# DreamWaterFound/self_commit_ORB-SLAM2

Hardware: AMD Instinct MI355X
Metric: frames/s ORB extract+match (1000 feat, 640x480) (higher is better)
Workload: dtype u8; 1 GPU; batch of 256 synthetic 640x480 frames per GPU (8 distinct resident batches per step, one launch set per batch), ORB extract (1000 feat, 8 levels, FAST 20/7) + brute-force Hamming SearchByBoW of consecutive frames; batch_per_gpu=256, streams=3, width=640, height=480, nfeatures=1000, parallelism=frames sharded, 1 rank(s), no data-path collective

## Files before the change

### self_commit_orb-slam2_amd/csrc/orbx_extractor.hip

```cpp
#include <math.h>
#include <stdarg.h>
#include <stdio.h>
#include <stdlib.h>
#include <string.h>

#include <algorithm>
#include <atomic>
#include <chrono>
#include <condition_variable>
#include <functional>
#include <memory>
#include <mutex>
#include <thread>
#include <vector>

#include "orbx_internal.h"

static thread_local char g_err[512] = "";

void orbx_set_error(const char *fmt, ...)
{
    va_list ap;
    va_start(ap, fmt);
    vsnprintf(g_err, sizeof(g_err), fmt, ap);
// ... 49 lines not shown
    hipStream_t stream = nullptr;
    hipEvent_t ev[ORBX_PROF_RING][ST_COUNT + 1] = {};
    bool profiling = false;
    int profCount = 0;
    bool debugTaps = false;
    DevBuf<OrbxGeom> geomDev;
    DevBuf<uint8_t> binDev, pyr, blur, score, staging;
    DevBuf<uint32_t> rsDev;
    DevBuf<OrbxFcCell> fcDev;
    DevBuf<int> cellCount, lvlCnt, lvlBase, status;
    DevBuf<uint8_t> outArena[2];
    int *outCntP[2] = {nullptr, nullptr};
    int *outStP[2] = {nullptr, nullptr};
    orbx_keypoint *outKpP[2] = {nullptr, nullptr};
    uint8_t *outDescP[2] = {nullptr, nullptr};
    size_t arenaKpOff = 0, arenaDescOff = 0, arenaBytes = 0;
    hipEvent_t consumerEv[2] = {nullptr, nullptr};
    hipEvent_t pyrConsumerEv = nullptr;
    int cur = 0;
    DevBuf<uint32_t> cellSlots, ptBuf, labBuf;
    DevBuf<OrbxLevelKp> lvlKp;
    int allocBatch = 0;
    int lastBatch = 0;
    bool lastChunked = false;
    const uint8_t *lastImg0 = nullptr;
    int lastStride = 0;
    size_t lastFramePitch = 0;
    uint8_t *hostStaging = nullptr;
    size_t hostStagingBytes = 0;
    int stagingStride = 0;
    size_t stagingFramePitch = 0;
    uint8_t *hostOut = nullptr;
    size_t hostOutBytes = 0;
    hipGraph_t sgGraph[2] = {nullptr, nullptr};
    hipGraphExec_t sgExec[2] = {nullptr, nullptr};
    bool sgValid = false;
    bool sgDisabled = false;
    struct Combiner *comb = nullptr;
    bool combDisabled = false;
    orbx_extractor *expectPartner = nullptr;
    bool isEngine = false;
    size_t hostPyrOff = 0;
    bool hostPyrValid = false;
    bool hostSynced = false;
    bool lastCombined = false;
    struct PipeSlot {
// ... 214 lines not shown
    g.fcPitch = maxWCell <= 32 ? 48 : maxWCell <= 48 ? 64 : 80;
    g.fcScPitch = maxWCell <= 42 ? 48 : 80;
    {
        int maxAw = 1;
        for (int l = 0; l < nl; l++) {
            const OrbxLevel &lv = g.lv[l];
            const int maxBX = lv.w - ORBX_BORDER;
            for (int cj = 0; cj < lv.nCols; cj++) {
                const int iniX = ORBX_BORDER + cj * lv.wCell, maxX = std::min(iniX + lv.wCell + 6, maxBX);
                maxAw = std::max(maxAw, (maxX - 3) - (iniX + 3));
            }
        }
        g.fcScPitch = maxAw + 2 <= 48 ? 48 : 80;
        if (g.fcScPitch == 80) g.fcPitch = 80;
    }
    { const char *pe = getenv("ORBX_FC_PITCH"); if (pe && atoi(pe) == 80 && g.fcPitch == 64) g.fcPitch = 80; }
    {
        const int units = (maxHCell + 6) * ((maxWCell + 6 + 15) / 16), ns = (units + 63) / 64;
        g.fcNS = ns <= 2 ? 2 : ns <= 3 ? 3 : ns <= 4 ? 4 : 6;
    }
    g.fcInBytes = g.fcPitch * (maxHCell + 6);
    g.fcScBytes = g.fcScPitch * (maxHCell + 2);
    g.fcLdsBytes = g.fcInBytes + g.fcScBytes + (int)align_up((size_t)maxWCell * maxHCell * 2, 16);
    h->fcHost.assign((size_t)cells, OrbxFcCell{});
    for (int l = 0; l < nl; l++) {
        const OrbxLevel &lv = g.lv[l];
        const int maxBX = lv.w - ORBX_BORDER, maxBY = lv.h - ORBX_BORDER;
        for (int ci = 0; ci < lv.nRows; ci++)
            for (int cj = 0; cj < lv.nCols; cj++) {
                const int cell = ci * lv.nCols + cj;
                OrbxFcCell &e = h->fcHost[(size_t)lv.cellBase + cell];
                const int iniX = ORBX_BORDER + cj * lv.wCell, iniY = ORBX_BORDER + ci * lv.hCell;
                const int maxX = std::min(iniX + lv.wCell + 6, maxBX), maxY = std::min(iniY + lv.hCell + 6, maxBY);
                const int x0 = iniX + 3, x1 = maxX - 3, y0 = iniY + 3, y1 = maxY - 3, aw = x1 - x0, ah = y1 - y0;
                const bool valid = !(iniY >= maxBY - 3 || iniX >= maxBX - 6 || aw <= 0 || ah <= 0);
                e.xy = valid ? ((uint32_t)x0 | ((uint32_t)y0 << 16)) : ((uint32_t)ORBX_EDGE | ((uint32_t)ORBX_EDGE << 16));
                const int ew = valid ? aw : 1, eh = valid ? ah : 1, nu = (ew + 6 + 15) / 16;
                e.dim = (uint32_t)ew | ((uint32_t)eh << 8) | ((uint32_t)l << 16) | (valid ? 1u << 24 : 0u);
                e.inv = (uint32_t)((65536 + nu - 1) / nu); e.units = (uint32_t)nu | ((uint32_t)((eh + 6) * nu) << 8);
                e.pitch = lv.pitch; e.off = (uint32_t)lv.off;
                e.slot = (uint32_t)(lv.slotBase + cell * lv.cellCap); e.cap = (uint32_t)lv.cellCap;
            }
    }
    g.pyrBytes = align_up(off + 256, 256);
    if (maxNodes > 2048) { orbx_set_error("per-level feature quota %d exceeds the quadtree node capacity 2048", maxNodes); return ORBX_ERR_ARG; }
    h->nodeCap = maxNodes <= 256 ? 256 : (maxNodes <= 512 ? 512 : (maxNodes <= 1024 ? 1024 : 2048));
// ... 100 lines not shown
    if (h->pyrConsumerEv) { ORBX_HIP_CHECK(hipStreamWaitEvent(h->stream, h->pyrConsumerEv, 0)); h->pyrConsumerEv = nullptr; }
    ORBX_HIP_CHECK(hipMemsetAsync(h->status.p, 0, (size_t)(batch + 1) * sizeof(int), h->stream));
    if (prof) ORBX_HIP_CHECK(hipEventRecord(ev[0], h->stream));
    static const bool batchTiles = getenv("ORBX_BATCH_PYR_TILES") && getenv("ORBX_BATCH_PYR_TILES")[0] == '1';
    bool tiled = false;
    if (batchTiles && h->allocBatch > 1) {
        if (h->ptBatchW != W || h->ptBatchH != H) {
            std::vector<OrbxPyrTile> plan;
            h->ptTiles = 0;
            if (plan_pyramid_tiles(h, plan, h->ptTiles, h->ptLds, h->ptTab)) {
                if ((rc = h->ptDev.ensure(plan.size())) != ORBX_OK) return rc;
                ORBX_HIP_CHECK(hipMemcpy(h->ptDev.p, plan.data(), plan.size() * sizeof(OrbxPyrTile), hipMemcpyHostToDevice));
            } else h->ptTiles = 0;
            h->ptBatchW = W; h->ptBatchH = H;
        }
        if (h->ptTiles > 0) {
            L.pyrTiles = h->ptDev.p; L.pyrTileCount = h->ptTiles; L.pyrTileBuf = h->ptLds; L.pyrTileTab = h->ptTab;
            if ((rc = orbx_launch_pyramid_tiles(L)) != ORBX_OK) return rc;
            tiled = true;
        }
    }
    const char *es = getenv("ORBX_PYR_SPLIT");
    L.pyrBand = !tiled && h->geom.pyrBand && !(es && es[0] == '1');
    if (L.pyrBand) {
        for (int l = 0; l < h->geom.nlevels; l++)
            if ((rc = orbx_launch_pyr_band(L, l)) != ORBX_OK) return rc;
    } else if (!tiled)
        for (int l = 1; l < h->geom.nlevels; l++)
            if ((rc = orbx_launch_resize(L, l)) != ORBX_OK) return rc;
    if (prof) ORBX_HIP_CHECK(hipEventRecord(ev[ST_PYR + 1], h->stream));
    if ((rc = orbx_launch_fast_cells(L)) != ORBX_OK) return rc;
    if (prof) ORBX_HIP_CHECK(hipEventRecord(ev[ST_FAST + 1], h->stream));
    if ((rc = orbx_launch_octree(L)) != ORBX_OK) return rc;
    if (prof) ORBX_HIP_CHECK(hipEventRecord(ev[ST_OCTREE + 1], h->stream));
    if (prof) ORBX_HIP_CHECK(hipEventRecord(ev[ST_ORIENT + 1], h->stream));
    if (!L.pyrBand && (rc = orbx_launch_blur(L)) != ORBX_OK) return rc;
    if (prof) ORBX_HIP_CHECK(hipEventRecord(ev[ST_BLUR + 1], h->stream));
    if (h->consumerEv[cb]) { ORBX_HIP_CHECK(hipStreamWaitEvent(h->stream, h->consumerEv[cb], 0)); h->consumerEv[cb] = nullptr; }
    if ((rc = orbx_launch_orient_describe(L)) != ORBX_OK) return rc;
    if (prof) { ORBX_HIP_CHECK(hipEventRecord(ev[ST_DESC + 1], h->stream)); h->profCount++; }
    h->lastBatch = batch; h->lastImg0 = img0Dev; h->lastStride = stride; h->lastFramePitch = framePitch;
    h->lastCombined = false; h->hostSynced = false; h->lastChunked = false;
    return ORBX_OK;
}

static int host_copy_threads()
{
    static const int n = [] {
        const char *e = getenv("ORBX_HOST_COPY_THREADS");
        int v = e && *e ? atoi(e) : (int)std::min(16u, std::max(1u, std::thread::hardware_concurrency() / 2));
        return v < 1 ? 1 : v > 64 ? 64 : v;
    }();
    return n;
}
struct CopyPool {
    std::mutex m;
    std::mutex jm;
    std::condition_variable cvWork, cvDone;
    std::vector<std::thread> workers;
    std::function<void(int, int)> job;
    int n = 0, parts = 0, gen = 0, pending = 0;
    bool stop = false;
    void worker(int id)
    {
        int seen = 0;
        for (;;) {
            std::function<void(int, int)> fn;
// ... 1514 lines not shown
```

### self_commit_orb-slam2_amd/csrc/orbx_internal.h

```cpp
#ifndef ORBX_INTERNAL_H
#define ORBX_INTERNAL_H

#include <hip/hip_runtime.h>
#include <cstring>
#include <stdint.h>

#include "../../include/orbx.h"

#define ORBX_MAX_LEVELS 12
#define ORBX_EDGE 19
#define ORBX_BORDER 16
#define ORBX_HALF_PATCH 15
#define ORBX_PATCH 31
#define ORBX_CELL_W 30
#define ORBX_MAX_INI 8

#define ORBX_DEV_ERR_PTCAP 1
#define ORBX_DEV_ERR_NODECAP 2
#define ORBX_DEV_ERR_KPCAP 4

struct OrbxLevel {
    int w, h, pitch;
    int off;
    int nCols, nRows, wCell, hCell;
// ... 4 lines not shown
    int nIni;
    int iniX[ORBX_MAX_INI + 1];
    int binOff;
    int kpBase, kpCap;
    int blurTileBase, blurTilesX, blurTilesY;
    int bandH, bandPitch;
    int bandOff;
    uint32_t bandDivNc, bandDivG4;
    double rsScaleX, rsScaleY;
    int rsColOff, rsRowOff;
    int patchSize;
    float scale;
};

struct OrbxGeom {
    int nlevels, W, H;
    int iniTh, minTh;
    int cellsPerFrame, slotsPerFrame, kpPerFrame, outCap;
    int blurTiles;
    int fcPitch, fcScPitch, fcNS;
    int fcInBytes, fcScBytes, fcLdsBytes;
    size_t pyrBytes;
    int pyrBand;
    uint32_t taps[7];
    int umax[16];
    OrbxLevel lv[ORBX_MAX_LEVELS];
};

#define ORBX_BAND_MAX_ITEMS (1 << 14)
static inline uint32_t orbx_band_div(int n)
{
    uint32_t S = 14;
    while ((1u << (S - 14)) < (uint32_t)n) S++;
    const uint32_t m = (uint32_t)((((uint64_t)1 << S) + (uint64_t)n - 1) / (uint64_t)n);
    return m | (S << 20);
}

struct OrbxFcCell {
    uint32_t xy;
    uint32_t dim;
    int32_t pitch;
    uint32_t off;
    uint32_t slot;
    uint32_t cap;
    uint32_t inv;
    uint32_t units;
};
#define ORBX_FC_CELLS_PER_WAVE 4

struct OrbxPyrTile { short cx0, cy0, cx1, cy1, ox0, oy0, ox1, oy1; };

struct OrbxCombMember {
    const uint8_t *srcImg;
    uint8_t *devImg;
    uint8_t *devPyr;
    uint8_t *devArena;
    uint8_t *hostOut;
    uint8_t *hostPyr;
// ... 4 lines not shown
void orbx_set_error(const char *fmt, ...);
#define ORBX_HIP_CHECK(expr)                                                                           \
    do {                                                                                               \
        hipError_t e_ = (expr);                                                                        \
        if (e_ != hipSuccess) {                                                                        \
            orbx_set_error("%s failed: %s (%s:%d)", #expr, hipGetErrorString(e_), __FILE__, __LINE__); \
            return ORBX_ERR_HIP;                                                                       \
        }                                                                                              \
    } while (0)

struct OrbxLaunch {
    hipStream_t stream;
    const OrbxGeom *geomDev;
    const OrbxGeom *geom;
    int batch;
    const uint8_t *img0;
    int img0Stride;
    size_t img0FramePitch;
    uint8_t *pyr, *blur, *score;
    size_t blurBytes;
    const uint8_t *binTab;
    const uint32_t *rsTab;
    const OrbxFcCell *fcCells;
    int *cellCount;
    uint32_t *cellSlots;
    uint32_t *ptBuf, *labBuf;
    OrbxLevelKp *lvlKp;
    int *lvlCnt;
    int *outBase;
    orbx_keypoint *outKp;
    uint8_t *outDesc;
    int *outCnt;
    int *status;
    int *outStatus;
    int nodeCap;
    bool pyrBand = false;
    const OrbxCombMember *combTab = nullptr;
    OrbxCombMember *combTabCopy = nullptr;
    unsigned *combSync = nullptr;
    unsigned long long *combFlag = nullptr;
    size_t combKpOff = 0, combDescOff = 0;
    const OrbxPyrTile *pyrTiles = nullptr; int pyrTileCount = 0, pyrTileBuf = 0, pyrTileTab = 0;
    hipGraph_t graph = nullptr;
    hipGraphNode_t deps[2] = {nullptr, nullptr};
    int ndeps = 0;
    hipGraphNode_t *node = nullptr;
};

int orbx_launch_resize(const OrbxLaunch &L, int level);
int orbx_launch_pyr_band(const OrbxLaunch &L, int level);
int orbx_launch_pyramid_tiles(const OrbxLaunch &L);
int orbx_launch_comb_upload(const OrbxLaunch &L, uint8_t *stagingDev);
int orbx_launch_comb_finish(const OrbxLaunch &L);
int orbx_launch_fast_cells(const OrbxLaunch &L);
int orbx_launch_octree(const OrbxLaunch &L);
int orbx_launch_blur(const OrbxLaunch &L);
int orbx_launch_octree_blur(const OrbxLaunch &L, bool *fused);
int orbx_launch_gather_frames(hipStream_t stream, const uint8_t *const *framesPinnedTab, int batch, int W, int H, int srcStride, uint8_t *dst, int dstStride, size_t framePitch, bool aligned16);
int orbx_launch_orient_describe(const OrbxLaunch &L);

hipStream_t orbx_extractor_stream_internal(orbx_extractor *h);
bool orbx_extractor_host_complete_internal(orbx_extractor *h, int *status);
int orbx_extractor_host_count_internal(orbx_extractor *h);
const orbx_keypoint *orbx_extractor_host_keypoints_internal(orbx_extractor *h);
void orbx_extractor_set_consumer_event_internal(orbx_extractor *h, hipEvent_t ev);
const int *orbx_extractor_status_word_internal(orbx_extractor *h);


template <typename T> struct OrbxDevBuf {
    T *p = nullptr;
    size_t n = 0;
    int ensure(size_t count)
    {
// ... 158 lines not shown
```

### self_commit_orb-slam2_amd/csrc/orbx_kernels.hip

```cpp
#include <algorithm>
#include "orbx_internal.h"

namespace {

struct OdTables {
    float pat[256][4];
    uint32_t disc[64][4];
};
constexpr int8_t kPattern[1024] = {
#include "orb_pattern.inc"
};
constexpr int kUmax[16] = {15, 15, 15, 15, 14, 14, 14, 13, 13, 12, 11, 10, 9, 8, 6, 3};
constexpr OdTables make_od_tables()
{
    OdTables t{};
    for (int i = 0; i < 256; i++) {
        t.pat[i][0] = (float)kPattern[4 * i]; t.pat[i][2] = (float)kPattern[4 * i + 1];
        t.pat[i][1] = (float)kPattern[4 * i + 2]; t.pat[i][3] = (float)kPattern[4 * i + 3];
    }
    for (int ml = 0; ml < 64; ml++)
        for (int j = 0; j < 4; j++) {
            const int mr = ml >> 1, mh = ml & 1;
            uint32_t m = 0u;
            if (mr < 31) {
// ... 271 lines not shown
                                            0x0c000c00u | (uint32_t)((b) & 3) | ((uint32_t)(((b) & 3) + 1) << 16))


#define FC_STAMP(i) do { if (PROF) { const unsigned long long t_ = __builtin_amdgcn_s_memtime(); pacc[i] += t_ - tPrev; tPrev = __builtin_amdgcn_s_memtime(); pacc[11] += tPrev - t_; } } while (0)

__device__ __forceinline__ uint4 load16u(const uint8_t *p)
{
    typedef uint32_t u32x4_u __attribute__((ext_vector_type(4), aligned(1)));
    const u32x4_u v = *(const u32x4_u *)p;
    return make_uint4(v.x, v.y, v.z, v.w);
}

__device__ __forceinline__ int wave_incl_scan_dpp(int v)
{
    v += __builtin_amdgcn_update_dpp(0, v, 0x111, 0xf, 0xf, false);
    v += __builtin_amdgcn_update_dpp(0, v, 0x112, 0xf, 0xf, false);
    v += __builtin_amdgcn_update_dpp(0, v, 0x114, 0xf, 0xf, false);
    v += __builtin_amdgcn_update_dpp(0, v, 0x118, 0xf, 0xf, false);
    v += __builtin_amdgcn_update_dpp(0, v, 0x142, 0xa, 0xf, false);
    v += __builtin_amdgcn_update_dpp(0, v, 0x143, 0xc, 0xf, false);
    return v;
}

template <int P, int SP, int NS, bool PROF = false, bool DBG = false>
__global__ __launch_bounds__(64) void k_fast_cells(const OrbxFcCell *__restrict__ cells, int K, int cellsPerFrame, int slotsPerFrame, size_t pyrBytes, int iniTh, int minTh,
                                                   int inBytes, int scBytes, const uint8_t *__restrict__ img0, int img0Stride, size_t img0FramePitch,
                                                   const uint8_t *__restrict__ pyr, uint8_t *__restrict__ scoreDbg, int *__restrict__ cellCount,
                                                   uint32_t *__restrict__ cellSlots, unsigned long long *__restrict__ prof)
{
    extern __shared__ __attribute__((aligned(16))) uint8_t lds[];
    uint8_t *inT = lds;
    uint8_t *scT = lds + inBytes;
    unsigned short *cand = (unsigned short *)(scT + scBytes);
    unsigned long long pacc[12] = {0, 0, 0, 0, 0, 0, 0, 0, 0, 0, 0, 0}, tPrev = 0;
    if (PROF) tPrev = __builtin_amdgcn_s_memtime();
    XCD_REMAP_XY(bx, f);
    const int lane = threadIdx.x;
    const int cFirst = bx * K, cEnd = min(cFirst + K, cellsPerFrame);
    const uint8_t *frame0 = img0 + (size_t)f * img0FramePitch, *frameP = pyr + (size_t)f * pyrBytes;
    uint4 wv[NS];
    int wo[NS], ur[NS], uc[NS];
    uint32_t shape = 0xffffffffu;
#define FC_REQUEST(E) do { \
        const int lvl_ = (int)(((E).dim >> 16) & 0xffu), sp_ = lvl_ ? (E).pitch : img0Stride; \
        const uint8_t *base_ = (lvl_ ? frameP + (E).off : frame0) + (size_t)((int)((E).xy >> 16) - 3) * sp_ + ((int)((E).xy & 0xffffu) - 3); \
        if ((E).units != shape) { \
            shape = (E).units; \
            const int nu_ = (int)((E).units & 0xffu), ntot_ = (int)((E).units >> 8), inv_ = (int)(E).inv; \
            _Pragma("unroll") for (int k_ = 0; k_ < NS; k_++) { \
                const int u_ = min(lane + 64 * k_, ntot_ - 1); \
                ur[k_] = __mul24(u_, inv_) >> 16; uc[k_] = 16 * (u_ - __mul24(ur[k_], nu_)); \
                wo[k_] = lane + 64 * k_ < ntot_ ? ur[k_] * P + uc[k_] : -1; \
            } \
        } \
        _Pragma("unroll") for (int k_ = 0; k_ < NS; k_++) wv[k_] = load16u(base_ + (size_t)ur[k_] * sp_ + uc[k_]); \
    } while (0)
    OrbxFcCell e = cells[cFirst], en = cells[min(cFirst + 1, cEnd - 1)];
    FC_REQUEST(e);
    FC_STAMP(0);
    for (int ci = cFirst; ci < cEnd; ci++) {
    int pNc1 = 0, pNc2 = 0, pRetry = 0;
    const int aw = (int)(e.dim & 0xffu), ah = (int)((e.dim >> 8) & 0xffu);
    const bool valid = (e.dim >> 24) != 0;
    const int x0 = (int)(e.xy & 0xffffu), y0 = (int)(e.xy >> 16);
    const int lpitch = e.pitch, cellCap = (int)e.cap;
    const uint32_t loff = e.off, slotOff = e.slot;
    int *cnt = cellCount + (size_t)f * cellsPerFrame + ci;
    {
#pragma unroll
        for (int k = 0; k < NS; k++)
            if (wo[k] >= 0) *(uint4 *)(inT + wo[k]) = wv[k];
        uint4 *z = (uint4 *)scT;
        for (int i = lane; i < (ah + 2) * (SP / 16); i += 64) z[i] = make_uint4(0u, 0u, 0u, 0u);
    }
    e = en;
    FC_REQUEST(e);
    en = cells[min(ci + 2, cEnd - 1)];
    if (!valid) {
        if (lane == 0) *cnt = 0;
        continue;
    }
    __syncthreads();
    FC_STAMP(1);
    uint8_t *dbg = DBG && scoreDbg ? scoreDbg + (size_t)f * pyrBytes + loff : nullptr;
    if (dbg)
        for (int p = lane; p < aw * ah; p += 64) dbg[(size_t)(y0 + p / aw) * lpitch + (x0 + p % aw)] = 0;

    const int S = (aw + 15) >> 4;
    const int rpp = S == 1 ? 64 : S == 2 ? 32 : S == 3 ? 21 : 16;
    const int rl = S == 1 ? lane : S == 2 ? (lane >> 1) : S == 3 ? ((lane * 43) >> 7) : (lane >> 2);
    const int seg = lane - rl * S, c0 = 16 * seg;
    const uint32_t colMask = (aw - c0 >= 16) ? 0xffffu : (aw - c0 <= 0 ? 0u : ((1u << (aw - c0)) - 1u));
    int nc = 0, th = dbg ? minTh : iniTh, base = 0;
    bool anyIni = false;
    uint32_t *slot = cellSlots + (size_t)f * slotsPerFrame + slotOff;
    for (;;) {
    nc = 0;
    const uint32_t thrPk = (uint32_t)(th & 0xffff) * 0x00010001u;
    for (int rowBase = 0; rowBase < ah; rowBase += rpp) {
        const int r = rowBase + rl;
        const bool live = rl < rpp && r < ah;
        const uint8_t *wp = inT + min(r, ah - 1) * P + c0;
        uint32_t W[7][6];
#pragma unroll
        for (int dy = 0; dy < 7; dy += 3) {
// ... 11 lines not shown
                const uint32_t xb = FC_PAIR(W[3 + FAST_DY(k + 8)], j + 3 + FAST_DX(k + 8));
                A = pk_max_u16(A, pk_min_u16(xa, xb));
                B = pk_min_u16(B, pk_max_u16(xa, xb));
            }
            const uint32_t vv = FC_PAIR(W[3], j + 3);
            const uint32_t m = pk_max_i16(pk_sub_i16(vv, A), pk_sub_i16(B, vv));
            mask |= ((pk_sub_i16(thrPk, m) >> 15) & 0x00010001u) << j;
        }
        mask = (mask & 0x5555u) | ((mask >> 15) & 0xaaaau);
        mask = live ? (mask & colMask) : 0u;
        if (PROF) { asm volatile("" :: "v"(mask)); FC_STAMP(th == iniTh || dbg ? 2 : 6); }
        const int cntL = __popc(mask);
        const int incl = wave_incl_scan_dpp(cntL);
        unsigned short *o = cand + (nc + incl - cntL);
        const int code0 = (r << 6) | c0;
        while (mask) {
            const int bpos = __ffs(mask) - 1;
            mask &= mask - 1;
            *o++ = (unsigned short)(code0 + bpos);
        }
        nc += __builtin_amdgcn_readlane(incl, 63);
        FC_STAMP(th == iniTh || dbg ? 3 : 7);
    }
    __syncthreads();
    if (PROF) { if (th == iniTh || dbg) pNc1 = nc; else { pNc2 = nc; pRetry = 1; } }

    for (int i = lane; i < nc; i += 64) {
        const int code = cand[i], r = code >> 6, c = code & 63;
        const uint8_t *q = inT + r * P + c;
        const int v = q[3 * P + 3];
        int x[16];
#pragma unroll
        for (int k = 0; k < 16; k++) x[k] = q[(3 + FAST_DY(k)) * P + 3 + FAST_DX(k)];
        int a3[16], b3[16];
#pragma unroll
        for (int k = 0; k < 16; k++) {
            a3[k] = min3u_asm(x[k], x[(k + 1) & 15], x[(k + 2) & 15]);
            b3[k] = max3u_asm(x[k], x[(k + 1) & 15], x[(k + 2) & 15]);
        }
        int maxA = 0, minB = 255;
#pragma unroll
        for (int k = 0; k < 16; k += 2) {
            const int a9 = min3u_asm(a3[k], a3[(k + 3) & 15], a3[(k + 6) & 15]), a9n = min3u_asm(a3[k + 1], a3[(k + 4) & 15], a3[(k + 7) & 15]);
            const int b9 = max3u_asm(b3[k], b3[(k + 3) & 15], b3[(k + 6) & 15]), b9n = max3u_asm(b3[k + 1], b3[(k + 4) & 15], b3[(k + 7) & 15]);
            maxA = k == 0 ? max(a9, a9n) : max3u_asm(maxA, a9, a9n);
            minB = k == 0 ? min(b9, b9n) : min3u_asm(minB, b9, b9n);
        }
        int sco = max(v - minB, maxA - v) - 1;
        sco = sco >= th ? sco : 0;
        scT[(r + 1) * SP + c + 4] = (uint8_t)sco;
        if (dbg) dbg[(size_t)(y0 + r) * lpitch + (x0 + c)] = (uint8_t)sco;
    }
    __syncthreads();
    FC_STAMP(th == iniTh || dbg ? 4 : 8);

    base = 0;
    anyIni = false;
    for (int i0 = 0; i0 < nc; i0 += 64) {
        const int i = i0 + lane;
        bool nms = false, ini = false;
        int code = 0, v = 0;
        if (i < nc) {
            code = cand[i];
            const int r = code >> 6, c = code & 63;
            const uint8_t *sp = scT + (r + 1) * SP + c + 4;
            v = sp[0];
            const int nb = max3i(max3i(sp[-1], sp[1], sp[-SP - 1]), max3i(sp[-SP], sp[-SP + 1], sp[SP - 1]), max(sp[SP], sp[SP + 1]));
            nms = v > nb;
            ini = nms && v >= iniTh;
        }
        if (dbg) {
            if (i < nc) cand[i] = (unsigned short)(code | (nms ? 0x1000 : 0) | (ini ? 0x2000 : 0));
            anyIni = anyIni || ini;
        } else {
            const unsigned long long m = __ballot(nms);
            if (nms) {
                const int r = code >> 6, c = code & 63;
                const int idx = base + __popcll(m & ((1ull << lane) - 1ull));
                if (idx < cellCap) slot[idx] = (uint32_t)(x0 + c - ORBX_BORDER) | ((uint32_t)(y0 + r - ORBX_BORDER) << 12) | ((uint32_t)v << 24);
            }
            base += __popcll(m);
        }
    }
    if (dbg) anyIni = __any(anyIni); else anyIni = base > 0;
    FC_STAMP(th == iniTh || dbg ? 5 : 9);
    if (anyIni || th == minTh) break;
    th = minTh;
    __syncthreads();
    }
    if (dbg) {
        const int keepBit = anyIni ? 0x2000 : 0x1000;
        base = 0;
        for (int i0 = 0; i0 < nc; i0 += 64) {
            const int i = i0 + lane;
            bool keep = false;
            int code = 0;
            if (i < nc) { code = cand[i]; keep = (code & keepBit) != 0; }
            const unsigned long long m = __ballot(keep);
            if (keep) {
                const int r = (code >> 6) & 63, c = code & 63;
                const uint32_t v = scT[(r + 1) * SP + c + 4];
                const int idx = base + __popcll(m & ((1ull << lane) - 1ull));
                if (idx < cellCap) slot[idx] = (uint32_t)(x0 + c - ORBX_BORDER) | ((uint32_t)(y0 + r - ORBX_BORDER) << 12) | (v << 24);
            }
            base += __popcll(m);
        }
    }
    if (lane == 0) *cnt = min(base, cellCap);
    __syncthreads();
    FC_STAMP(10);
    if (PROF && lane == 0) {
        unsigned long long *rec = prof + 32 + ((size_t)f * cellsPerFrame + ci) * 16;
        for (int i = 0; i < 12; i++) { rec[i] = pacc[i]; pacc[i] = 0; }
        rec[12] = (unsigned long long)pRetry; rec[13] = (unsigned long long)pNc1; rec[14] = (unsigned long long)pNc2; rec[15] = (unsigned long long)min(base, cellCap);
    }
    }
}
#undef FC_STAMP
#undef FC_REQUEST

struct OtBox { short x0, y0, x1, y1; };

template <typename T> __device__ __forceinline__ T wave_incl_scan(T v, int lane)
{
#pragma unroll
    for (int o = 1; o < 64; o <<= 1) {
        T u = __shfl_up(v, o);
        if (lane >= o) v += u;
    }
    return v;
}

template <int BT = 256, typename T> __device__ T block_exscan(T *arr, int n, T *wsum )
{
    const int tid = threadIdx.x, lane = tid & 63, w = tid >> 6;
    const int per = (n + BT - 1) / BT;
    const int b = tid * per;
    T s = 0;
    for (int k = 0; k < per; k++) if (b + k < n) s += arr[b + k];
    T inc = wave_incl_scan(s, lane);
    if (lane == 63) wsum[w] = inc;
    __syncthreads();
// ... 498 lines not shown
            const int r = pb_div(it, divNc), c = it - (int)__umul24((uint32_t)r, (uint32_t)nc);
            int y = s0 - 3 + r;
            if (EDGE) {
                y = reflect101(y, h);
                y = min(max(y, 0), h - 1);
            }
            const uint8_t *row = src + (size_t)y * sp;
            const int x = 16 * c;
            if (x + 16 <= readable) __builtin_memcpy(&v[k], row + x, 16);
            else {
                uint32_t t[4] = {0u, 0u, 0u, 0u};
                for (int j = 0; x + j < w; j++) t[j >> 2] |= (uint32_t)row[x + j] << (8 * (j & 3));
                v[k] = make_uint4(t[0], t[1], t[2], t[3]);
            }
            dOff[k] = item < items ? (int)__umul24((uint32_t)r, (uint32_t)P) + PB_ORG + x : -1;
        }
#pragma unroll
        for (int k = 0; k < PB_STAGE; k++)
            if (dOff[k] >= 0) *(uint4 *)(bb + dOff[k]) = v[k];
    }
}

template <bool CLAMP>
__global__ __launch_bounds__(PB_THREADS) void k_pyr_band(const OrbxGeom *__restrict__ g, const int l, const uint8_t *__restrict__ img0, int img0Stride, size_t img0FramePitch,
                                                         const int readable, uint8_t *__restrict__ pyr, uint8_t *__restrict__ blur, const uint32_t *__restrict__ rsTab,
                                                         int *__restrict__ outBase)
{
    extern __shared__ __attribute__((aligned(16))) uint32_t band[];
    uint8_t *bb = (uint8_t *)band;
    XCD_REMAP_XY(b, f);
    const int nl = g->nlevels, tid = (int)threadIdx.x;
    if (l == 0 && b == 0 && tid < nl && outBase) outBase[f * nl + tid] = 0;
    const OrbxLevel &lv = g->lv[l];
    const int w = lv.w, h = lv.h, P = lv.bandPitch;
    const int s0 = b * lv.bandH, s1 = min(s0 + lv.bandH, h);
    const int nr = ((s1 - s0 + 7) & ~7) + 6;
    int sp;
    const uint8_t *src = level_ptr(g, l, f, img0, img0Stride, img0FramePitch, pyr, sp);
    if (s0 >= 3 && s0 - 3 + nr <= h) pb_stage<false>(bb, src, sp, readable, w, h, P, s0, nr, lv.bandDivNc, tid);
    else pb_stage<true>(bb, src, sp, readable, w, h, P, s0, nr, lv.bandDivNc, tid);
    __syncthreads();
    for (int r = tid; r < nr; r += PB_THREADS) {
        uint8_t *rowb = bb + r * P + PB_ORG;
        rowb[-1] = rowb[1]; rowb[-2] = rowb[2]; rowb[-3] = rowb[3];
#pragma unroll
        for (int k = 0; k < 3; k++) rowb[w + k] = rowb[w - 2 - k];
    }
    __syncthreads();
    {
        const int G4 = (w + 3) >> 2, items = G4 * ((s1 - s0 + 7) >> 3), PW = P >> 2;
        const uint32_t pitch = (uint32_t)lv.pitch;
        const bool full = ((s1 - s0) & 7) == 0;
        uint8_t *dst = blur + (size_t)f * g->pyrBytes + lv.off;
// ... 64 lines not shown
            if (y0 != ra) {
                if (y0 == rb) {
#pragma unroll
                    for (int k = 0; k < 4; k++) ha[k] = hb[k];
                } else hpass(y0, ha);
                ra = y0;
            }
            if (y1 != rb) {
                if (y1 == ra) {
#pragma unroll
                    for (int k = 0; k < 4; k++) hb[k] = ha[k];
                } else hpass(y1, hb);
                rb = y1;
            }
            const uint32_t b0 = (t.y << 12) & 0x00fff000u, b1 = (t.y >> 4) & 0x00fff000u;
            uint32_t out = 0;
#pragma unroll
            for (int k = 0; k < 4; k++) out |= ((pb_mulhi24(b0, ha[k]) + pb_mulhi24(b1, hb[k]) + 2u) >> 2) << (8 * k);
            *(uint32_t *)(dstBase + o) = out;
        }
    }
}

#define OB_THREADS 1024
template <int NODECAP, bool CLAMP>
__global__ __launch_bounds__(OB_THREADS) void k_octree_blur(const OrbxGeom *__restrict__ g, const int *__restrict__ cellCount, const uint32_t *__restrict__ cellSlots,
                                                     const uint8_t *__restrict__ binTab, uint32_t *__restrict__ ptBuf, uint32_t *__restrict__ labBuf,
                                                     OrbxLevelKp *__restrict__ lvlKp, int *__restrict__ lvlCnt, int *__restrict__ status,
                                                     const OrbxCombMember *__restrict__ comb, const uint8_t *__restrict__ img0, int img0Stride, size_t img0FramePitch,
                                                     uint8_t *__restrict__ pyr, uint8_t *__restrict__ blur)
{
    extern __shared__ __attribute__((aligned(16))) uint32_t blurLds[];
    const int bx = (int)blockIdx.x, f = (int)blockIdx.y, nl = g->nlevels;
    if (bx < nl) { octree_body<NODECAP, OB_THREADS>(g, cellCount, cellSlots, binTab, ptBuf, labBuf, lvlKp, lvlCnt, status, bx, f, (int)gridDim.y); return; }
    if (bx < nl + ORBX_OCTREE_COPY_BLOCKS) { host_pyramid_copy(g, comb, pyr, f, bx - nl, ORBX_OCTREE_COPY_BLOCKS); return; }
    const int wv = (int)(threadIdx.x >> 6), tile = __builtin_amdgcn_readfirstlane((bx - nl - ORBX_OCTREE_COPY_BLOCKS) * (OB_THREADS / 64) + wv);
    blur_body<CLAMP>(g, img0, img0Stride, img0FramePitch, pyr, blur, min(tile, g->blurTiles - 1), f, blurLds + wv * (BT_IH * (BT_P / 4)), (int)(threadIdx.x & 63), tile < g->blurTiles);
}

__device__ __forceinline__ int wave_sum_dpp(int v)
{
    v += __builtin_amdgcn_update_dpp(0, v, 0xb1, 0xf, 0xf, true);
    v += __builtin_amdgcn_update_dpp(0, v, 0x4e, 0xf, 0xf, true);
    v += __builtin_amdgcn_update_dpp(0, v, 0x141, 0xf, 0xf, true);
    v += __builtin_amdgcn_update_dpp(0, v, 0x140, 0xf, 0xf, true);
    v += __builtin_amdgcn_update_dpp(0, v, 0x142, 0xa, 0xf, true);
// ... 292 lines not shown
    }
    return emit(L, k_pyramid_tiles, dim3((unsigned)L.pyrTileCount, (unsigned)L.batch), dim3(256), ldsBytes, L.geomDev, L.img0, L.img0Stride, L.img0FramePitch, L.pyr, L.rsTab,
                L.pyrTiles, L.pyrTileBuf, L.status);
}

int orbx_launch_comb_upload(const OrbxLaunch &L, uint8_t *stagingDev)
{
    const size_t units = L.img0FramePitch >> 4;
    const unsigned blocks = (unsigned)std::min<size_t>(std::max<size_t>((units + 255) / 256, 1), 256);
    return emit(L, k_comb_upload, dim3(blocks, (unsigned)L.batch), dim3(256), 0, L.combTab, L.combTabCopy, stagingDev, L.img0FramePitch);
}

int orbx_launch_comb_finish(const OrbxLaunch &L)
{
    const size_t units = (L.geom->pyrBytes + L.img0FramePitch) >> 4;
    const unsigned blocks = (unsigned)std::min<size_t>(std::max<size_t>((units + 2047) / 2048, 1), 64);
    return emit(L, k_comb_finish, dim3(blocks, (unsigned)L.batch), dim3(256), 0, (const OrbxCombMember *)L.combTabCopy, L.outCnt, L.outStatus, L.outKp, L.outDesc, L.geom->outCap, L.pyr, L.geom->pyrBytes, L.img0,
                L.img0FramePitch, L.combKpOff, L.combDescOff, 0, L.combSync, L.combFlag);
}

static unsigned long long *g_fcProf = nullptr;
extern "C" void orbx_debug_fast_cells_profile(unsigned long long *dev32) { g_fcProf = dev32; }

int orbx_launch_fast_cells(const OrbxLaunch &L)
{
    const OrbxGeom &g = *L.geom;
    static const int kEnv = getenv("ORBX_FC_CELLS_PER_WAVE") ? atoi(getenv("ORBX_FC_CELLS_PER_WAVE")) : 0;
    const int K = kEnv > 0 ? kEnv : (L.batch >= 32 ? ORBX_FC_CELLS_PER_WAVE : 1);
    dim3 grid((unsigned)((g.cellsPerFrame + K - 1) / K), (unsigned)L.batch);
    const size_t ldsBytes = (size_t)g.fcLdsBytes;
#define FC_ARGS L.fcCells, K, g.cellsPerFrame, g.slotsPerFrame, g.pyrBytes, g.iniTh, g.minTh, g.fcInBytes, g.fcScBytes, L.img0, L.img0Stride, L.img0FramePitch, L.pyr, L.score, L.cellCount, L.cellSlots
#define FC_LAUNCH(PP, SS, NN) do { if (L.score) return emit(L, k_fast_cells<PP, SS, NN, false, true>, grid, dim3(64), ldsBytes, FC_ARGS, (unsigned long long *)nullptr); \
    if (g_fcProf) return emit(L, k_fast_cells<PP, SS, NN, true, false>, grid, dim3(64), ldsBytes, FC_ARGS, g_fcProf); \
    return emit(L, k_fast_cells<PP, SS, NN, false, false>, grid, dim3(64), ldsBytes, FC_ARGS, (unsigned long long *)nullptr); } while (0)
#define FC_LAUNCH_P(PP, SS) switch (g.fcNS) { case 2: FC_LAUNCH(PP, SS, 2); case 3: FC_LAUNCH(PP, SS, 3); case 4: FC_LAUNCH(PP, SS, 4); default: FC_LAUNCH(PP, SS, 6); }
    if (g.fcPitch == 48 && g.fcScPitch == 48) FC_LAUNCH_P(48, 48)
    if (g.fcPitch == 64 && g.fcScPitch == 48) FC_LAUNCH_P(64, 48)
    if (g.fcPitch == 80 && g.fcScPitch == 48) FC_LAUNCH_P(80, 48)
    if (g.fcPitch != 80 || g.fcScPitch != 80) { orbx_set_error("detector LDS pitches %d / %d have no kernel instantiation", g.fcPitch, g.fcScPitch); return ORBX_ERR_STATE; }
    FC_LAUNCH_P(80, 80)
#undef FC_LAUNCH_P
#undef FC_LAUNCH
#undef FC_ARGS
}

int orbx_launch_octree(const OrbxLaunch &L)
{
    dim3 grid((unsigned)(L.geom->nlevels + (L.combTab ? ORBX_OCTREE_COPY_BLOCKS : 0)), (unsigned)L.batch);
#define OT_LAUNCH(NC) return emit(L, k_octree<NC>, grid, dim3(256), 0, L.geomDev, L.cellCount, L.cellSlots, L.binTab, L.ptBuf, L.labBuf, L.lvlKp, L.lvlCnt, L.status, L.combTab, \
                                  (const uint8_t *)L.pyr, L.pyrBand ? L.outBase : (int *)nullptr)
    if (L.nodeCap <= 256) OT_LAUNCH(256);
    if (L.nodeCap <= 512) OT_LAUNCH(512);
    if (L.nodeCap <= 1024) OT_LAUNCH(1024);
    OT_LAUNCH(2048);
// ... 33 lines not shown

int orbx_launch_blur(const OrbxLaunch &L)
{
    dim3 grid((unsigned)L.geom->blurTiles, (unsigned)L.batch);
    unsigned tapSum = 0;
    for (int i = 0; i < 7; i++) tapSum += L.geom->taps[i];
    if (tapSum > 256u) return emit(L, k_blur<true>, grid, dim3(64), 0, L.geomDev, L.img0, L.img0Stride, L.img0FramePitch, L.pyr, L.blur, L.lvlCnt, L.outBase);
    return emit(L, k_blur<false>, grid, dim3(64), 0, L.geomDev, L.img0, L.img0Stride, L.img0FramePitch, L.pyr, L.blur, L.lvlCnt, L.outBase);
}

int orbx_launch_pyr_band(const OrbxLaunch &L, int l)
{
    const OrbxGeom &g = *L.geom;
    const OrbxLevel &lv = g.lv[l];
    const dim3 grid((unsigned)((lv.h + lv.bandH - 1) / lv.bandH), (unsigned)L.batch);
    const size_t lds = (size_t)(lv.bandH + 6) * lv.bandPitch;
    const int readable = l > 0 ? lv.pitch : (L.img0FramePitch >= (size_t)L.img0Stride * (size_t)lv.h ? L.img0Stride : lv.w);
    unsigned tapSum = 0;
    for (int i = 0; i < 7; i++) tapSum += g.taps[i];
    if (tapSum > 256u) return emit(L, k_pyr_band<true>, grid, dim3(PB_THREADS), lds, L.geomDev, l, L.img0, L.img0Stride, L.img0FramePitch, readable, L.pyr, L.blur, L.rsTab, L.outBase);
    return emit(L, k_pyr_band<false>, grid, dim3(PB_THREADS), lds, L.geomDev, l, L.img0, L.img0Stride, L.img0FramePitch, readable, L.pyr, L.blur, L.rsTab, L.outBase);
}

int orbx_launch_orient_describe(const OrbxLaunch &L)
{
    dim3 grid((unsigned)((L.geom->kpPerFrame + OD_WPB - 1) / OD_WPB), (unsigned)L.batch);
    const OrbxGeom &g = *L.geom;
    OdLevels A;
    memset(&A, 0, sizeof(A));
    A.nlevels = g.nlevels; A.kpPerFrame = g.kpPerFrame; A.outCap = g.outCap; A.pyrBytes = g.pyrBytes;
    for (int l = 0; l < ORBX_MAX_LEVELS; l++) A.kpBase[l] = 0x7fffffff;
    for (int l = 0; l < g.nlevels; l++) { A.kpBase[l] = g.lv[l].kpBase; A.off[l] = g.lv[l].off; A.pitch[l] = g.lv[l].pitch; A.patch[l] = g.lv[l].patchSize; A.scale[l] = g.lv[l].scale; }
    for (int i = 0; i < 16; i++)
        if (g.umax[i] != kUmax[i]) { orbx_set_error("disc half-widths differ from the compiled table"); return ORBX_ERR_STATE; }
    return emit(L, k_orient_describe, grid, dim3(64 * OD_WPB), 0, A, L.img0, L.img0Stride, L.img0FramePitch, L.pyr, L.blur, L.lvlKp, L.lvlCnt, L.combTab ? (const int *)nullptr : (const int *)L.outBase, L.outKp, L.outDesc,
                L.outCnt, L.status, L.outStatus);
}
```

Measured before the change: 310,400 frames/s.

## Fuse FAST cell detection for top pyramid levels into pyramid band kernel

Adds a combined kernel that runs the pyramid band work for a level alongside extra blocks. Each extra block holds four waves, and each wave runs FAST corner detection on that level's cells. This applies to the first two levels, and the separate FAST launch then covers only the remaining levels. The goal is to overlap detection with pyramid construction and cut launches and tail idle time. Block-wide barriers in the FAST body become wave-level fences so several independent waves can share a block. The catch is a larger LDS allocation for band blocks, which may lower occupancy, and a reliance on the level data being ready before it is read within the same launch.

```diff
diff --git a/self_commit_orb-slam2_amd/csrc/orbx_extractor.hip b/self_commit_orb-slam2_amd/csrc/orbx_extractor.hip
--- a/self_commit_orb-slam2_amd/csrc/orbx_extractor.hip
+++ b/self_commit_orb-slam2_amd/csrc/orbx_extractor.hip
@@ -95,6 +95,7 @@
     DevBuf<OrbxLevelKp> lvlKp;
     int allocBatch = 0;
     int lastBatch = 0;
+    bool lastPyrFast = false;
     bool lastChunked = false;
     const uint8_t *lastImg0 = nullptr;
     int lastStride = 0;
@@ -355,6 +356,7 @@
     g.fcInBytes = g.fcPitch * (maxHCell + 6);
     g.fcScBytes = g.fcScPitch * (maxHCell + 2);
     g.fcLdsBytes = g.fcInBytes + g.fcScBytes + (int)align_up((size_t)maxWCell * maxHCell * 2, 16);
+    g.pyrFast = g.pyrBand && (size_t)ORBX_PF_WAVES * (size_t)g.fcLdsBytes <= 48 * 1024 ? 1 : 0;
     h->fcHost.assign((size_t)cells, OrbxFcCell{});
     for (int l = 0; l < nl; l++) {
         const OrbxLevel &lv = g.lv[l];
@@ -501,14 +503,18 @@
     }
     const char *es = getenv("ORBX_PYR_SPLIT");
     L.pyrBand = !tiled && h->geom.pyrBand && !(es && es[0] == '1');
+    const char *ef = getenv("ORBX_FAST_SPLIT");
+    const bool pyrFast = L.pyrBand && orbx_pyr_fast_applies(L) && !(ef && ef[0] == '1');
+    const int nJoin = pyrFast ? std::min(ORBX_PF_JOIN_LEVELS, h->geom.nlevels) : 0;
     if (L.pyrBand) {
         for (int l = 0; l < h->geom.nlevels; l++)
-            if ((rc = orbx_launch_pyr_band(L, l)) != ORBX_OK) return rc;
+            if ((rc = l < nJoin ? orbx_launch_pyr_band_fast(L, l) : orbx_launch_pyr_band(L, l)) != ORBX_OK) return rc;
     } else if (!tiled)
         for (int l = 1; l < h->geom.nlevels; l++)
             if ((rc = orbx_launch_resize(L, l)) != ORBX_OK) return rc;
     if (prof) ORBX_HIP_CHECK(hipEventRecord(ev[ST_PYR + 1], h->stream));
-    if ((rc = orbx_launch_fast_cells(L)) != ORBX_OK) return rc;
+    L.fcCellFirst = nJoin < h->geom.nlevels ? h->geom.lv[nJoin].cellBase : h->geom.cellsPerFrame;
+    if (L.fcCellFirst < h->geom.cellsPerFrame && (rc = orbx_launch_fast_cells(L)) != ORBX_OK) return rc;
     if (prof) ORBX_HIP_CHECK(hipEventRecord(ev[ST_FAST + 1], h->stream));
     if ((rc = orbx_launch_octree(L)) != ORBX_OK) return rc;
     if (prof) ORBX_HIP_CHECK(hipEventRecord(ev[ST_OCTREE + 1], h->stream));
@@ -519,9 +525,11 @@
     if ((rc = orbx_launch_orient_describe(L)) != ORBX_OK) return rc;
     if (prof) { ORBX_HIP_CHECK(hipEventRecord(ev[ST_DESC + 1], h->stream)); h->profCount++; }
     h->lastBatch = batch; h->lastImg0 = img0Dev; h->lastStride = stride; h->lastFramePitch = framePitch;
-    h->lastCombined = false; h->hostSynced = false; h->lastChunked = false;
-    return ORBX_OK;
-}
+    h->lastCombined = false; h->hostSynced = false; h->lastChunked = false; h->lastPyrFast = pyrFast;
+    return ORBX_OK;
+}
+
+extern "C" int orbx_debug_last_batch_pyr_fast(orbx_extractor *h) { return h && h->lastPyrFast ? 1 : 0; }
 
 static int host_copy_threads()
 {
diff --git a/self_commit_orb-slam2_amd/csrc/orbx_internal.h b/self_commit_orb-slam2_amd/csrc/orbx_internal.h
--- a/self_commit_orb-slam2_amd/csrc/orbx_internal.h
+++ b/self_commit_orb-slam2_amd/csrc/orbx_internal.h
@@ -50,6 +50,7 @@
     int fcInBytes, fcScBytes, fcLdsBytes;
     size_t pyrBytes;
     int pyrBand;
+    int pyrFast;
     uint32_t taps[7];
     int umax[16];
     OrbxLevel lv[ORBX_MAX_LEVELS];
@@ -62,6 +63,15 @@
     while ((1u << (S - 14)) < (uint32_t)n) S++;
     const uint32_t m = (uint32_t)((((uint64_t)1 << S) + (uint64_t)n - 1) / (uint64_t)n);
     return m | (S << 20);
+}
+
+#define ORBX_PF_WAVES 4
+#define ORBX_PF_JOIN_LEVELS 2
+static inline int orbx_fast_blocks(int cells, int K) { return (cells + ORBX_PF_WAVES * K - 1) / (ORBX_PF_WAVES * K); }
+static inline size_t orbx_pyr_fast_lds(const OrbxGeom &g, int l)
+{
+    const size_t band = (size_t)(g.lv[l].bandH + 6) * (size_t)g.lv[l].bandPitch, fast = (size_t)ORBX_PF_WAVES * (size_t)g.fcLdsBytes;
+    return band > fast ? band : fast;
 }
 
 struct OrbxFcCell {
@@ -112,6 +122,7 @@
     const uint8_t *binTab;
     const uint32_t *rsTab;
     const OrbxFcCell *fcCells;
+    int fcCellFirst = 0;
     int *cellCount;
     uint32_t *cellSlots;
     uint32_t *ptBuf, *labBuf;
@@ -139,6 +150,8 @@
 
 int orbx_launch_resize(const OrbxLaunch &L, int level);
 int orbx_launch_pyr_band(const OrbxLaunch &L, int level);
+bool orbx_pyr_fast_applies(const OrbxLaunch &L);
+int orbx_launch_pyr_band_fast(const OrbxLaunch &L, int level);
 int orbx_launch_pyramid_tiles(const OrbxLaunch &L);
 int orbx_launch_comb_upload(const OrbxLaunch &L, uint8_t *stagingDev);
 int orbx_launch_comb_finish(const OrbxLaunch &L);
diff --git a/self_commit_orb-slam2_amd/csrc/orbx_kernels.hip b/self_commit_orb-slam2_amd/csrc/orbx_kernels.hip
--- a/self_commit_orb-slam2_amd/csrc/orbx_kernels.hip
+++ b/self_commit_orb-slam2_amd/csrc/orbx_kernels.hip
@@ -317,21 +317,24 @@
     return v;
 }
 
-template <int P, int SP, int NS, bool PROF = false, bool DBG = false>
-__global__ __launch_bounds__(64) void k_fast_cells(const OrbxFcCell *__restrict__ cells, int K, int cellsPerFrame, int slotsPerFrame, size_t pyrBytes, int iniTh, int minTh,
-                                                   int inBytes, int scBytes, const uint8_t *__restrict__ img0, int img0Stride, size_t img0FramePitch,
-                                                   const uint8_t *__restrict__ pyr, uint8_t *__restrict__ scoreDbg, int *__restrict__ cellCount,
-                                                   uint32_t *__restrict__ cellSlots, unsigned long long *__restrict__ prof)
-{
-    extern __shared__ __attribute__((aligned(16))) uint8_t lds[];
+__device__ __forceinline__ void fc_wave_sync()
+{
+    __builtin_amdgcn_fence(__ATOMIC_RELEASE, "workgroup");
+    __builtin_amdgcn_wave_barrier();
+    __builtin_amdgcn_fence(__ATOMIC_ACQUIRE, "workgroup");
+}
+
+template <int P, int SP, int NS, bool PROF, bool DBG>
+__device__ __forceinline__ void fast_cells_body(const OrbxFcCell *__restrict__ cells, const int cFirst, const int cEnd, const int f, uint8_t *__restrict__ lds, const int lane,
+                                                int cellsPerFrame, int slotsPerFrame, size_t pyrBytes, int iniTh, int minTh,
+                                                int inBytes, int scBytes, const uint8_t *__restrict__ img0, int img0Stride, size_t img0FramePitch,
+                                                const uint8_t *__restrict__ pyr, uint8_t *__restrict__ scoreDbg, int *__restrict__ cellCount,
+                                                uint32_t *__restrict__ cellSlots, unsigned long long *__restrict__ prof, unsigned long long tStart)
+{
     uint8_t *inT = lds;
     uint8_t *scT = lds + inBytes;
     unsigned short *cand = (unsigned short *)(scT + scBytes);
-    unsigned long long pacc[12] = {0, 0, 0, 0, 0, 0, 0, 0, 0, 0, 0, 0}, tPrev = 0;
-    if (PROF) tPrev = __builtin_amdgcn_s_memtime();
-    XCD_REMAP_XY(bx, f);
-    const int lane = threadIdx.x;
-    const int cFirst = bx * K, cEnd = min(cFirst + K, cellsPerFrame);
+    unsigned long long pacc[12] = {0, 0, 0, 0, 0, 0, 0, 0, 0, 0, 0, 0}, tPrev = tStart;
     const uint8_t *frame0 = img0 + (size_t)f * img0FramePitch, *frameP = pyr + (size_t)f * pyrBytes;
     uint4 wv[NS];
     int wo[NS], ur[NS], uc[NS];
@@ -375,7 +378,7 @@
         if (lane == 0) *cnt = 0;
         continue;
     }
-    __syncthreads();
+    fc_wave_sync();
     FC_STAMP(1);
     uint8_t *dbg = DBG && scoreDbg ? scoreDbg + (size_t)f * pyrBytes + loff : nullptr;
     if (dbg)
@@ -433,7 +436,7 @@
         nc += __builtin_amdgcn_readlane(incl, 63);
         FC_STAMP(th == iniTh || dbg ? 3 : 7);
     }
-    __syncthreads();
+    fc_wave_sync();
     if (PROF) { if (th == iniTh || dbg) pNc1 = nc; else { pNc2 = nc; pRetry = 1; } }
 
     for (int i = lane; i < nc; i += 64) {
@@ -462,7 +465,7 @@
         scT[(r + 1) * SP + c + 4] = (uint8_t)sco;
         if (dbg) dbg[(size_t)(y0 + r) * lpitch + (x0 + c)] = (uint8_t)sco;
     }
-    __syncthreads();
+    fc_wave_sync();
     FC_STAMP(th == iniTh || dbg ? 4 : 8);
 
     base = 0;
@@ -497,7 +500,7 @@
     FC_STAMP(th == iniTh || dbg ? 5 : 9);
     if (anyIni || th == minTh) break;
     th = minTh;
-    __syncthreads();
+    fc_wave_sync();
     }
     if (dbg) {
         const int keepBit = anyIni ? 0x2000 : 0x1000;
@@ -518,7 +521,7 @@
         }
     }
     if (lane == 0) *cnt = min(base, cellCap);
-    __syncthreads();
+    fc_wave_sync();
     FC_STAMP(10);
     if (PROF && lane == 0) {
         unsigned long long *rec = prof + 32 + ((size_t)f * cellsPerFrame + ci) * 16;
@@ -529,6 +532,21 @@
 }
 #undef FC_STAMP
 #undef FC_REQUEST
+
+template <int P, int SP, int NS, bool PROF = false, bool DBG = false>
+__global__ __launch_bounds__(64) void k_fast_cells(const OrbxFcCell *__restrict__ cells, int cell0, int K, int cellsPerFrame, int slotsPerFrame, size_t pyrBytes, int iniTh, int minTh,
+                                                   int inBytes, int scBytes, const uint8_t *__restrict__ img0, int img0Stride, size_t img0FramePitch,
+                                                   const uint8_t *__restrict__ pyr, uint8_t *__restrict__ scoreDbg, int *__restrict__ cellCount,
+                                                   uint32_t *__restrict__ cellSlots, unsigned long long *__restrict__ prof)
+{
+    extern __shared__ __attribute__((aligned(16))) uint8_t lds[];
+    unsigned long long tStart = 0;
+    if (PROF) tStart = __builtin_amdgcn_s_memtime();
+    XCD_REMAP_XY(bx, f);
+    const int cFirst = cell0 + bx * K;
+    fast_cells_body<P, SP, NS, PROF, DBG>(cells, cFirst, min(cFirst + K, cellsPerFrame), f, lds, (int)threadIdx.x, cellsPerFrame, slotsPerFrame, pyrBytes, iniTh, minTh, inBytes, scBytes,
+                                          img0, img0Stride, img0FramePitch, pyr, scoreDbg, cellCount, cellSlots, prof, tStart);
+}
 
 struct OtBox { short x0, y0, x1, y1; };
 
@@ -1073,13 +1091,11 @@
 }
 
 template <bool CLAMP>
-__global__ __launch_bounds__(PB_THREADS) void k_pyr_band(const OrbxGeom *__restrict__ g, const int l, const uint8_t *__restrict__ img0, int img0Stride, size_t img0FramePitch,
-                                                         const int readable, uint8_t *__restrict__ pyr, uint8_t *__restrict__ blur, const uint32_t *__restrict__ rsTab,
-                                                         int *__restrict__ outBase)
-{
-    extern __shared__ __attribute__((aligned(16))) uint32_t band[];
+__device__ __forceinline__ void pyr_band_body(const OrbxGeom *__restrict__ g, const int l, const uint8_t *__restrict__ img0, int img0Stride, size_t img0FramePitch,
+                                              const int readable, uint8_t *__restrict__ pyr, uint8_t *__restrict__ blur, const uint32_t *__restrict__ rsTab,
+                                              int *__restrict__ outBase, const int b, const int f, uint32_t *__restrict__ band)
+{
     uint8_t *bb = (uint8_t *)band;
-    XCD_REMAP_XY(b, f);
     const int nl = g->nlevels, tid = (int)threadIdx.x;
     if (l == 0 && b == 0 && tid < nl && outBase) outBase[f * nl + tid] = 0;
     const OrbxLevel &lv = g->lv[l];
@@ -1190,6 +1206,36 @@
     }
 }
 
+template <bool CLAMP>
+__global__ __launch_bounds__(PB_THREADS) void k_pyr_band(const OrbxGeom *__restrict__ g, const int l, const uint8_t *__restrict__ img0, int img0Stride, size_t img0FramePitch,
+                                                         const int readable, uint8_t *__restrict__ pyr, uint8_t *__restrict__ blur, const uint32_t *__restrict__ rsTab,
+                                                         int *__restrict__ outBase)
+{
+    extern __shared__ __attribute__((aligned(16))) uint32_t band[];
+    XCD_REMAP_XY(b, f);
+    pyr_band_body<CLAMP>(g, l, img0, img0Stride, img0FramePitch, readable, pyr, blur, rsTab, outBase, b, f, band);
+}
+
+template <bool CLAMP, int P, int SP, int NS>
+__global__ __launch_bounds__(PB_THREADS) void k_pyr_band_fast(const OrbxGeom *__restrict__ g, const int l, const uint8_t *__restrict__ img0, int img0Stride, size_t img0FramePitch,
+                                                              const int readable, uint8_t *__restrict__ pyr, uint8_t *__restrict__ blur, const uint32_t *__restrict__ rsTab,
+                                                              int *__restrict__ outBase, const int nBands, const OrbxFcCell *__restrict__ cells, const int K, const int cellLo,
+                                                              const int cellHi, int cellsPerFrame, int slotsPerFrame, size_t pyrBytes, int iniTh, int minTh, int inBytes, int scBytes,
+                                                              const int fcLds, int *__restrict__ cellCount, uint32_t *__restrict__ cellSlots)
+{
+    extern __shared__ __attribute__((aligned(16))) uint32_t band[];
+    XCD_REMAP_XY(bx, f);
+    if (bx < nBands) {
+        pyr_band_body<CLAMP>(g, l, img0, img0Stride, img0FramePitch, readable, pyr, blur, rsTab, outBase, bx, f, band);
+        return;
+    }
+    const int wv = __builtin_amdgcn_readfirstlane((int)(threadIdx.x >> 6));
+    const int cFirst = cellLo + (((bx - nBands) * (PB_THREADS / 64) + wv) * K);
+    if (cFirst >= cellHi) return;
+    fast_cells_body<P, SP, NS, false, false>(cells, cFirst, min(cFirst + K, cellHi), f, (uint8_t *)band + wv * fcLds, (int)(threadIdx.x & 63), cellsPerFrame, slotsPerFrame, pyrBytes, iniTh,
+                                             minTh, inBytes, scBytes, img0, img0Stride, img0FramePitch, pyr, nullptr, cellCount, cellSlots, nullptr, 0ull);
+}
+
 #define OB_THREADS 1024
 template <int NODECAP, bool CLAMP>
 __global__ __launch_bounds__(OB_THREADS) void k_octree_blur(const OrbxGeom *__restrict__ g, const int *__restrict__ cellCount, const uint32_t *__restrict__ cellSlots,
@@ -1528,14 +1574,19 @@
 static unsigned long long *g_fcProf = nullptr;
 extern "C" void orbx_debug_fast_cells_profile(unsigned long long *dev32) { g_fcProf = dev32; }
 
+static int fc_cells_per_wave(int batch)
+{
+    static const int kEnv = getenv("ORBX_FC_CELLS_PER_WAVE") ? atoi(getenv("ORBX_FC_CELLS_PER_WAVE")) : 0;
+    return kEnv > 0 ? kEnv : (batch >= 32 ? ORBX_FC_CELLS_PER_WAVE : 1);
+}
+
 int orbx_launch_fast_cells(const OrbxLaunch &L)
 {
     const OrbxGeom &g = *L.geom;
-    static const int kEnv = getenv("ORBX_FC_CELLS_PER_WAVE") ? atoi(getenv("ORBX_FC_CELLS_PER_WAVE")) : 0;
-    const int K = kEnv > 0 ? kEnv : (L.batch >= 32 ? ORBX_FC_CELLS_PER_WAVE : 1);
-    dim3 grid((unsigned)((g.cellsPerFrame + K - 1) / K), (unsigned)L.batch);
+    const int K = fc_cells_per_wave(L.batch);
+    dim3 grid((unsigned)((g.cellsPerFrame - L.fcCellFirst + K - 1) / K), (unsigned)L.batch);
     const size_t ldsBytes = (size_t)g.fcLdsBytes;
-#define FC_ARGS L.fcCells, K, g.cellsPerFrame, g.slotsPerFrame, g.pyrBytes, g.iniTh, g.minTh, g.fcInBytes, g.fcScBytes, L.img0, L.img0Stride, L.img0FramePitch, L.pyr, L.score, L.cellCount, L.cellSlots
+#define FC_ARGS L.fcCells, L.fcCellFirst, K, g.cellsPerFrame, g.slotsPerFrame, g.pyrBytes, g.iniTh, g.minTh, g.fcInBytes, g.fcScBytes, L.img0, L.img0Stride, L.img0FramePitch, L.pyr, L.score, L.cellCount, L.cellSlots
 #define FC_LAUNCH(PP, SS, NN) do { if (L.score) return emit(L, k_fast_cells<PP, SS, NN, false, true>, grid, dim3(64), ldsBytes, FC_ARGS, (unsigned long long *)nullptr); \
     if (g_fcProf) return emit(L, k_fast_cells<PP, SS, NN, true, false>, grid, dim3(64), ldsBytes, FC_ARGS, g_fcProf); \
     return emit(L, k_fast_cells<PP, SS, NN, false, false>, grid, dim3(64), ldsBytes, FC_ARGS, (unsigned long long *)nullptr); } while (0)
@@ -1615,6 +1666,34 @@
     return emit(L, k_pyr_band<false>, grid, dim3(PB_THREADS), lds, L.geomDev, l, L.img0, L.img0Stride, L.img0FramePitch, readable, L.pyr, L.blur, L.rsTab, L.outBase);
 }
 
+bool orbx_pyr_fast_applies(const OrbxLaunch &L) { return L.geom->pyrBand && L.geom->pyrFast && !L.score && !g_fcProf; }
+
+int orbx_launch_pyr_band_fast(const OrbxLaunch &L, int l)
+{
+    const OrbxGeom &g = *L.geom;
+    const OrbxLevel &lv = g.lv[l];
+    const int K = fc_cells_per_wave(L.batch), ncell = lv.nCols * lv.nRows;
+    const int nBands = (lv.h + lv.bandH - 1) / lv.bandH;
+    const dim3 grid((unsigned)(nBands + orbx_fast_blocks(ncell, K)), (unsigned)L.batch);
+    const size_t lds = orbx_pyr_fast_lds(g, l);
+    const int readable = l > 0 ? lv.pitch : (L.img0FramePitch >= (size_t)L.img0Stride * (size_t)lv.h ? L.img0Stride : lv.w);
+    unsigned tapSum = 0;
+    for (int i = 0; i < 7; i++) tapSum += g.taps[i];
+#define PF_ARGS L.geomDev, l, L.img0, L.img0Stride, L.img0FramePitch, readable, L.pyr, L.blur, L.rsTab, L.outBase, nBands, L.fcCells, K, lv.cellBase, lv.cellBase + ncell, g.cellsPerFrame, \
+                g.slotsPerFrame, g.pyrBytes, g.iniTh, g.minTh, g.fcInBytes, g.fcScBytes, g.fcLdsBytes, L.cellCount, L.cellSlots
+#define PF_LAUNCH(PP, SS, NN) do { if (tapSum > 256u) return emit(L, k_pyr_band_fast<true, PP, SS, NN>, grid, dim3(PB_THREADS), lds, PF_ARGS); \
+    return emit(L, k_pyr_band_fast<false, PP, SS, NN>, grid, dim3(PB_THREADS), lds, PF_ARGS); } while (0)
+#define PF_LAUNCH_P(PP, SS) switch (g.fcNS) { case 2: PF_LAUNCH(PP, SS, 2); case 3: PF_LAUNCH(PP, SS, 3); case 4: PF_LAUNCH(PP, SS, 4); default: PF_LAUNCH(PP, SS, 6); }
+    if (g.fcPitch == 48 && g.fcScPitch == 48) PF_LAUNCH_P(48, 48)
+    if (g.fcPitch == 64 && g.fcScPitch == 48) PF_LAUNCH_P(64, 48)
+    if (g.fcPitch == 80 && g.fcScPitch == 48) PF_LAUNCH_P(80, 48)
+    if (g.fcPitch != 80 || g.fcScPitch != 80) { orbx_set_error("detector LDS pitches %d / %d have no kernel instantiation", g.fcPitch, g.fcScPitch); return ORBX_ERR_STATE; }
+    PF_LAUNCH_P(80, 80)
+#undef PF_LAUNCH_P
+#undef PF_LAUNCH
+#undef PF_ARGS
+}
+
 int orbx_launch_orient_describe(const OrbxLaunch &L)
 {
     dim3 grid((unsigned)((L.geom->kpPerFrame + OD_WPB - 1) / OD_WPB), (unsigned)L.batch);
```

New measurement: 318,500 frames/s, median of 6. +2.6%, better.
